# imjaegyun/Traffic-Context-Augmented-Vehicle-Trajectory-Prediction-Framework-Using-Multimodal-LLM

Hardware: AMD Instinct MI355X
Metric: trajectories/sec (higher is better)
Workload: dtype f16; 1 GPU; train.py step (:1168-1183): zero_grad + MultiModalTrajectoryModel.forward incl. loss (:914-964) + backward through the trainable part (LTSF + lane-polygon encoder; MLLM frozen, :1140-1145) + gradient all-reduce + AdamW(lr 5e-4, wd 1e-4); Llama-3.2-1B shape + LoRA r=8 + Q-Former + LTSF cross-attention head; dropout on as under ddp_model.train() (in-kernel Philox masks, regenerated in the backward); mode=train, variant=train.py (MLLM frozen), per_gpu_batch=32, global_batch=32, fused_seq_len=256, t_in=18, t_out=30, lora_r=8, parallelism=dp1, launch=eager

## Files before the change

traffic-context-augmented-vehicle-trajectory-prediction-framework-using-multimodal-llm_amd/csrc/gemm_bf16.hip:

```cpp
#include "gemm_params.hpp"
#include "gemm_epilogue.hpp"
#include "gemm_tile8.hpp"
#include "gemm_w4.hpp"
#include "gemm_skinny.hpp"
#include "gemm_splitk.hpp"

namespace tcavt {

template <int EPI, bool F16>
static int launch_small(const GemmP& p, int tile, int batch, hipStream_t stream) {
  GemmP q = p;
  q.prio = 0;
  const long wgs = (long)((q.M + 127) / 128) * ((q.N + 127) / 128) * batch;
  static const bool no_deep = getenv("TCAVT_GEMM_NO_DEEP") != nullptr;
  static const bool no_64 = getenv("TCAVT_GEMM_NO_64") != nullptr;
  if constexpr (EPI != EPI_ROPE && EPI != EPI_NORM && EPI != EPI_NORM16) {
    if ((tile == 64 || (tile == 0 && wgs <= 128 && !no_64)) && !no_deep) return launch<64, 64, 2, 2, EPI, F16, 2>(q, batch, stream);
  }
  if (wgs <= 256 && !no_deep) return launch<128, 128, 2, 2, EPI, F16, 2>(q, batch, stream);
  return launch<128, 128, 2, 2, EPI, F16, 1>(q, batch, stream);
}

template <int EPI, bool F16>
static int dispatch_tile(const GemmP& p, int tile, int batch, hipStream_t stream) {
// ... 51 lines not shown
}

extern "C" int tcavt_gemm_bf16(const tcavt_gemm_args* a, tcavt_stream_t stream) {
  TCAVT_CHECK_ARG(a != nullptr, "gemm_bf16: null args");
  const bool stream16 = (a->epilogue & TCAVT_EPI_NORM_OUT) && a->C == nullptr;
  TCAVT_CHECK_ARG(a->A && a->W && (a->C || stream16), "gemm_bf16: null A/W/C");
  TCAVT_CHECK_ARG(a->M > 0 && a->N > 0 && a->K > 0, "gemm_bf16: bad M/N/K %d/%d/%d", a->M, a->N, a->K);
  TCAVT_CHECK_ARG(a->K % 64 == 0, "gemm_bf16: K=%d must be a multiple of 64", a->K);
  TCAVT_CHECK_ARG(a->K < (1 << 26), "gemm_bf16: K too large");
  TCAVT_CHECK_ARG(a->N % 16 == 0, "gemm_bf16: N=%d must be a multiple of 16", a->N);
  TCAVT_CHECK_ARG(a->lda % 8 == 0 && a->ldw % 8 == 0 && a->lda >= a->K && a->ldw >= a->K,
                  "gemm_bf16: lda/ldw must be >= K and multiples of 8");
  TCAVT_CHECK_ARG(aligned16(a->A) && aligned16(a->W) && aligned16(a->C), "gemm_bf16: A/W/C must be 16-byte aligned");
  TCAVT_CHECK_ARG(a->out_dtype == TCAVT_F32 || a->out_dtype == TCAVT_BF16 || a->out_dtype == TCAVT_F16,
                  "gemm_bf16: bad out_dtype");
  TCAVT_CHECK_ARG(a->in_dtype == 0 || a->in_dtype == TCAVT_BF16 || a->in_dtype == TCAVT_F16, "gemm_bf16: bad in_dtype");
  const bool f16 = a->in_dtype == TCAVT_F16;
  const int batch = a->batch > 1 ? a->batch : 1;
  if (batch > 1)
    TCAVT_CHECK_ARG(!(a->epilogue & (TCAVT_EPI_SILU_MUL | TCAVT_EPI_ROPE)),
                    "gemm_bf16: batching is supported by the generic epilogue only");
  if (batch > 1) {
    TCAVT_CHECK_ARG(a->batch_inner >= 1 && batch % a->batch_inner == 0, "gemm_bf16: batch must be a multiple of batch_inner");
    TCAVT_CHECK_ARG(a->sAo % 8 == 0 && a->sAi % 8 == 0 && a->sWo % 8 == 0 && a->sWi % 8 == 0 && a->sCo % 4 == 0 &&
                        a->sCi % 4 == 0 && batch <= 65535,
                    "gemm_bf16: batch strides must keep 16-byte (A/W) and 4-element (C) alignment; batch <= 65535");
  }
  const int n_out = (a->epilogue & TCAVT_EPI_SILU_MUL) ? a->N / 2 : a->N;
  TCAVT_CHECK_ARG(a->ldc >= n_out && a->ldc % 4 == 0, "gemm_bf16: ldc=%ld too small or not a multiple of 4", (long)a->ldc);
  int K2 = 0;
  const bool lp_consumer = a->lora_part && (a->epilogue & TCAVT_EPI_ROPE);
  if ((a->A2 || a->W2 || a->K2) && !lp_consumer) {
    TCAVT_CHECK_ARG(a->A2 && a->W2 && a->K2 > 0 && a->K2 % 64 == 0,
                    "gemm_bf16: second K-source needs A2, W2 and K2 %% 64 == 0");
    TCAVT_CHECK_ARG(a->lda2 % 8 == 0 && a->ldw2 % 8 == 0 && a->lda2 >= a->K2 && a->ldw2 >= a->K2 &&
                        aligned16(a->A2) && aligned16(a->W2),
                    "gemm_bf16: bad lda2/ldw2/alignment");
    K2 = a->K2;
  }
  int epi = a->epilogue;
  if (epi & TCAVT_EPI_BIAS) TCAVT_CHECK_ARG(a->bias && aligned16(a->bias), "gemm_bf16: BIAS needs an aligned bias pointer");
  if (epi & TCAVT_EPI_BIAS_ROW) TCAVT_CHECK_ARG(a->bias && !(epi & TCAVT_EPI_BIAS), "gemm_bf16: BIAS_ROW needs bias and excludes BIAS");
  if ((epi & TCAVT_EPI_RESIDUAL) && !stream16)
    TCAVT_CHECK_ARG(a->residual && aligned16(a->residual) && a->ldr >= a->N && a->ldr % 4 == 0,
                    "gemm_bf16: RESIDUAL needs residual pointer and ldr >= N");
  if (epi & TCAVT_EPI_SILU_MUL)
    TCAVT_CHECK_ARG(a->N % 128 == 0 && !(epi & ~(TCAVT_EPI_SILU_MUL | TCAVT_EPI_ROWSCALE)),
                    "gemm_bf16: SILU_MUL needs N %% 128 == 0 and no other flag but ROWSCALE");
  if (epi & TCAVT_EPI_ROPE) {
    TCAVT_CHECK_ARG(a->N % 128 == 0 && !(epi & ~(TCAVT_EPI_ROPE | TCAVT_EPI_ROWSCALE)),
                    "gemm_bf16: ROPE needs N %% 128 == 0 and no other flag but ROWSCALE");
    TCAVT_CHECK_ARG(a->rope_cos && a->rope_sin && a->rope_L > 0 && a->rope_cols % 64 == 0 &&
                        aligned16(a->rope_cos) && aligned16(a->rope_sin),
                    "gemm_bf16: ROPE needs cos/sin tables, rope_L > 0, rope_cols %% 64 == 0");
  }
  TCAVT_CHECK_ARG(a->tile == 0 || a->tile == 64 || a->tile == 128 || a->tile == 256 || a->tile == 257 || a->tile == 271 || a->tile == 272,
                  "gemm_bf16: tile must be 0 (auto), 64, 128, 256, 257, 271 or 272");

  GemmP p;
  p.A = static_cast<const bf16_t*>(a->A);
  p.W = static_cast<const bf16_t*>(a->W);
  p.A2 = static_cast<const bf16_t*>(a->A2);
  p.W2 = static_cast<const bf16_t*>(a->W2);
  p.C = a->C;
  p.bias = a->bias;
  p.residual = a->residual;
  p.cosT = a->rope_cos;
  p.sinT = a->rope_sin;
  p.lda = a->lda; p.ldw = a->ldw; p.lda2 = a->lda2; p.ldw2 = a->ldw2; p.ldc = a->ldc; p.ldr = a->ldr;
  p.M = a->M; p.N = a->N; p.K = a->K; p.K2 = K2;
  p.out_kind = a->out_dtype;
  p.batch_inner = batch > 1 ? a->batch_inner : 1;
  p.w_group = a->batch_w_group > 1 ? a->batch_w_group : 1;
  p.sAo = a->sAo; p.sAi = a->sAi; p.sWo = a->sWo; p.sWi = a->sWi; p.sCo = a->sCo; p.sCi = a->sCi;
  p.flags = epi;
  p.rope_L = a->rope_L; p.rope_cols = a->rope_cols;
  p.tiles_m = p.tiles_n = 0;
  p.prio = 0;
  p.pers_tiles = 0;
  p.xcd_gx = 8;
  p.norm_h16 = nullptr;
  p.norm_part = nullptr;
  p.res16 = nullptr;
  p.lp_part = nullptr;
  p.lp_a = nullptr;
  p.lp_lda = 0;
  p.lp_np = 0;
  p.lp_scale = 1.f;
  p.w_frag = p.a_frag = p.o_frag = 0;
  if (a->act_layout != 0) {
    TCAVT_CHECK_ARG((a->act_layout & ~(TCAVT_ACT_A_FRAG16 | TCAVT_ACT_OUT_FRAG16 | TCAVT_ACT_BLOCK8)) == 0 && a->tile == 0 &&
                        skinny_shape(a->M, a->K) && batch == 1 && a->dropout_p == 0.f,
                    "gemm_bf16: act_layout (fragment-major activations) goes with the skinny form only (M <= 32, K %% 256 == 0, tile 0)");
    const int fmode = (a->act_layout & TCAVT_ACT_BLOCK8) ? 2 : 1;
    TCAVT_CHECK_ARG(fmode == 1 || a->M <= 8, "gemm_bf16: TCAVT_ACT_BLOCK8 holds at most 8 rows");
    p.a_frag = (a->act_layout & TCAVT_ACT_A_FRAG16) ? fmode : 0;
    if (a->act_layout & TCAVT_ACT_OUT_FRAG16) {
      const bool silu = (a->epilogue & ~TCAVT_EPI_ROWSCALE) == TCAVT_EPI_SILU_MUL && a->out_dtype == (f16 ? TCAVT_F16 : TCAVT_BF16) &&
                        a->N % 64 == 0;
      const bool stream = (a->epilogue & TCAVT_EPI_NORM_OUT) && stream16 && a->N % 32 == 0;
      TCAVT_CHECK_ARG(silu || stream, "gemm_bf16: TCAVT_ACT_OUT_FRAG16 needs SILU_MUL with a 16-bit output of the operand type, or "
                                      "NORM_OUT with C == NULL (the in-place 16-bit stream)");
      p.o_frag = fmode;
    }
  }
  if (a->w_layout != 0) {
    TCAVT_CHECK_ARG((a->w_layout == TCAVT_W_FRAG16 || a->w_layout == TCAVT_W_FRAG8) && a->tile == 0 && skinny_shape(a->M, a->K) && batch == 1 &&
                        a->dropout_p == 0.f && a->lda >= a->K && a->ldw == a->K && a->N % 16 == 0,
                    "gemm_bf16: w_layout = TCAVT_W_FRAG16 / TCAVT_W_FRAG8 (tcavt_pack_weight16 / tcavt_pack_weight8 copy) goes with the "
                    "skinny form only (M <= 32, K %% 256 == 0, N %% 16 == 0, tile 0, ldw == K)");
    p.w_frag = a->w_layout == TCAVT_W_FRAG8 ? 2 : 1;
  }
  if (a->lora_part) {
    TCAVT_CHECK_ARG(a->tile == 0 && skinny_shape(a->M, a->K) && batch == 1 && a->dropout_p == 0.f && aligned16(a->lora_part),
                    "gemm_bf16: lora_part goes with the skinny form only (M <= 32, tile 0)");
    p.lp_part = static_cast<float*>(a->lora_part);
    if (epi & TCAVT_EPI_NORM_OUT) {
      TCAVT_CHECK_ARG(a->lora_part_a && a->lora_part_lda >= a->N && a->lora_part_lda % 4 == 0 && ((uintptr_t)a->lora_part_a & 7) == 0,
                      "gemm_bf16: lora_part with NORM_OUT needs lora_part_a [32, lda >= N]");
      p.lp_a = static_cast<const bf16_t*>(a->lora_part_a);
      p.lp_lda = a->lora_part_lda;
    } else {
      TCAVT_CHECK_ARG((epi & TCAVT_EPI_ROPE) && a->lora_part_np > 0 && a->W2 && !a->A2 && a->K2 == 0 && a->ldw2 >= 32 && a->ldw2 % 8 == 0 &&
                          aligned16(a->W2) && a->M * 16 <= 512,
                      "gemm_bf16: lora_part with ROPE needs lora_part_np > 0, W2 (ldw2 >= 32) and no A2");
      p.lp_np = a->lora_part_np;
      p.lp_scale = a->lora_part_scale;
      p.W2 = static_cast<const bf16_t*>(a->W2);
      p.ldw2 = a->ldw2;
    }
  }
  p.sk_msplit = 1;
  p.sk_split = 1;
  p.sk_slab = nullptr;
  p.sk_cnt = nullptr;
  p.sk_slab_bytes = 0;
  p.sk_cnt_n = 0;
  if (a->splitk_ws && a->splitk_ws_bytes >= (64 << 10)) {
    TCAVT_CHECK_ARG(aligned16(a->splitk_ws), "gemm_bf16: splitk_ws must be 16-byte aligned");
    p.sk_cnt = static_cast<int*>(a->splitk_ws);
    p.sk_cnt_n = 4096;
    p.sk_slab = reinterpret_cast<float*>(static_cast<char*>(a->splitk_ws) + (16 << 10));
    p.sk_slab_bytes = a->splitk_ws_bytes - (16 << 10);
  }
  p.nf_flag = (epi & TCAVT_EPI_NORM_OUT) ? a->nonfinite_flag : nullptr;
  p.nf_tag = a->nonfinite_tag;
  p.norm_scale = 1.f;
  if (epi & TCAVT_EPI_NORM_OUT) {
    TCAVT_CHECK_ARG(a->norm_scale >= 0.f && a->norm_scale <= 1.f, "gemm_bf16: norm_scale must be in (0, 1] (0 means 1)");
    if (a->norm_scale != 0.f) p.norm_scale = a->norm_scale;
  }
  p.rs_part = nullptr;
  p.rope_pos = (epi & TCAVT_EPI_ROPE) ? a->rope_pos : nullptr;
  p.rs_npart = 0;
  p.rs_eps = p.rs_inv_h = 0.f;
  if (epi & TCAVT_EPI_NORM_OUT) {
    TCAVT_CHECK_ARG(!(epi & ~(TCAVT_EPI_NORM_OUT | TCAVT_EPI_RESIDUAL)) && a->out_dtype == TCAVT_F32 && batch == 1 && K2 == 0 &&
                        a->N % 64 == 0 && a->norm_h16 && a->norm_part && aligned16(a->norm_h16) && a->dropout_p == 0.f &&
                        (a->acc_scale == 0.f || a->acc_scale == 1.f) && a->tile != 64,
                    "gemm_bf16: NORM_OUT goes with an fp32 output (+ RESIDUAL) only, N %% 64 == 0, and needs norm_h16 / norm_part");
    TCAVT_CHECK_ARG(!stream16 || a->residual == nullptr,
                    "gemm_bf16: NORM_OUT with C == NULL keeps the residual stream in norm_h16 (updated in place): residual must be NULL");
    p.norm_h16 = static_cast<bf16_t*>(a->norm_h16);
    p.norm_part = a->norm_part;
    TCAVT_CHECK_ARG(a->norm_res16 == nullptr || (stream16 && aligned16(a->norm_res16)),
                    "gemm_bf16: norm_res16 goes with the 16-bit residual stream (NORM_OUT, C == NULL) and needs 16-byte alignment");
// ... 109 lines not shown
```

traffic-context-augmented-vehicle-trajectory-prediction-framework-using-multimodal-llm_amd/csrc/gemm_epilogue.hpp:

```cpp
#pragma once
#include "gemm_params.hpp"

namespace tcavt {

__device__ __forceinline__ void store_quad(const GemmP& p, int m, int n, f32x4 v) {
  if (p.out_kind == TCAVT_BF16) {
    u32x2 o = {pack_bf16x2(v[0], v[1]), pack_bf16x2(v[2], v[3])};
    *reinterpret_cast<u32x2*>(reinterpret_cast<bf16_t*>(p.C) + (long)m * p.ldc + n) = o;
  } else if (p.out_kind == TCAVT_F16) {
    u32x2 o = {pack_f16x2(v[0], v[1]), pack_f16x2(v[2], v[3])};
    *reinterpret_cast<u32x2*>(reinterpret_cast<bf16_t*>(p.C) + (long)m * p.ldc + n) = o;
  } else {
    *reinterpret_cast<f32x4*>(reinterpret_cast<float*>(p.C) + (long)m * p.ldc + n) = v;
  }
}

__device__ __forceinline__ float silu_mul(float g, float u) {
  return g * __builtin_amdgcn_rcpf(1.f + __expf(-g)) * u;
}

typedef __attribute__((ext_vector_type(2))) float f32x2;

template <bool F16>
__device__ __forceinline__ u32x2 silu_mul_quad(const f32x4& g, const f32x4& u) {
  const f32x2 g0 = {g[0], g[1]}, g1 = {g[2], g[3]}, u0 = {u[0], u[1]}, u1 = {u[2], u[3]};
  const f32x2 t0 = g0 * -1.44269504088896340736f, t1 = g1 * -1.44269504088896340736f;
  const f32x2 d0 = f32x2{__builtin_amdgcn_exp2f(t0[0]), __builtin_amdgcn_exp2f(t0[1])} + 1.f;
  const f32x2 d1 = f32x2{__builtin_amdgcn_exp2f(t1[0]), __builtin_amdgcn_exp2f(t1[1])} + 1.f;
  const f32x2 r0 = {__builtin_amdgcn_rcpf(d0[0]), __builtin_amdgcn_rcpf(d0[1])};
  const f32x2 r1 = {__builtin_amdgcn_rcpf(d1[0]), __builtin_amdgcn_rcpf(d1[1])};
  const f32x2 o0 = g0 * r0 * u0, o1 = g1 * r1 * u1;
  return u32x2{pack16x2<F16>(o0[0], o0[1]), pack16x2<F16>(o1[0], o1[1])};
}

__device__ __forceinline__ void swap16(unsigned& a, unsigned& b) {
  const auto r = __builtin_amdgcn_permlane16_swap(a, b, false, false);
  a = r[0];
  b = r[1];
}
__device__ __forceinline__ int pair16_off(int lane) {
  const int q = lane >> 4;
  return (q & 1) ? 16 + 4 * (q - 1) : 4 * q;
}
__device__ __forceinline__ void store_pair16(bf16_t* row_pair, int off, const u32x2& a, const u32x2& b) {
  unsigned a0 = a[0], a1 = a[1], b0 = b[0], b1 = b[1];
  swap16(a0, b0);
  swap16(a1, b1);
  *reinterpret_cast<u32x4*>(row_pair + off) = u32x4{a0, a1, b0, b1};
}
__device__ __forceinline__ void unswap_pair16(const u32x4& v, u32x2& a, u32x2& b) {
  unsigned a0 = v[0], a1 = v[1], b0 = v[2], b1 = v[3];
  swap16(a0, b0);
  swap16(a1, b1);
  a = u32x2{a0, a1};
  b = u32x2{b0, b1};
}

template <int TN, int TM>
__device__ __forceinline__ void pin_acc(f32x4 (&acc)[TN][TM], int i, int j) {
  asm volatile("" : "+a"(acc[i][j]));
}
template <int TM, int TN, int EPI, bool WHOLE_ONLY = false, bool F16 = false>
__device__ __forceinline__ void gemm_epilogue(const GemmP& p, f32x4 (&acc)[TN][TM], int m_base, int n_base, int lane,
                                              const float* rs_lds = nullptr) {
  constexpr int OUT16 = F16 ? TCAVT_F16 : TCAVT_BF16;
  float rsv[TM];
  if constexpr (EPI == EPI_SILU || EPI == EPI_SILU_SAVE || EPI == EPI_ROPE) {
    if (rs_lds) {
#pragma unroll
      for (int j = 0; j < TM; ++j) rsv[j] = rs_lds[j * 16 + (lane & 15)];
    } else if (p.rs_part) {
      float ss[TM];
      const f32x4* q[TM];
#pragma unroll
      for (int j = 0; j < TM; ++j) {
        ss[j] = 0.f;
        q[j] = reinterpret_cast<const f32x4*>(p.rs_part + (long)min(m_base + j * 16 + (lane & 15), p.M - 1) * p.rs_npart);
      }
      for (int i = 0; i < (p.rs_npart >> 2); ++i) {
#pragma unroll
        for (int j = 0; j < TM; ++j) {
          const f32x4 v = q[j][i];
          ss[j] += v[0];
          ss[j] += v[1];
          ss[j] += v[2];
          ss[j] += v[3];
        }
      }
#pragma unroll
      for (int j = 0; j < TM; ++j) rsv[j] = rsqrtf(ss[j] * p.rs_inv_h + p.rs_eps);
    } else {
#pragma unroll
      for (int j = 0; j < TM; ++j) rsv[j] = 1.f;
    }
  }
  const int nq = 4 * (lane >> 4);
  const int ml = lane & 15;
  const bool whole = WHOLE_ONLY || (m_base + TM * 16 <= p.M && n_base + TN * 16 <= p.N);
  if constexpr ((EPI == EPI_NORM || EPI == EPI_NORM16) && TN % 4 == 0) {
    const bool res = p.flags & TCAVT_EPI_RESIDUAL;
    const int npart = p.N >> 6;
    if constexpr (EPI == EPI_NORM16) {
      if constexpr (WHOLE_ONLY) {
        constexpr int DW = TM > 5 ? 5 : TM;
        const int off16 = pair16_off(lane);
        u32x4 oldw[TM][TN / 2];
        auto fetchw = [&](int j) {
          const bf16_t* hrow = p.res16 + (long)(m_base + j * 16 + ml) * p.ldc + n_base + off16;
#pragma unroll
          for (int k = 0; k < TN / 2; ++k)
            oldw[j][k] = res ? *reinterpret_cast<const u32x4*>(hrow + k * 32) : u32x4{0u, 0u, 0u, 0u};
        };
#pragma unroll
        for (int j = 0; j < DW; ++j) fetchw(j);
#pragma unroll
        for (int j = 0; j < TM; ++j) {
          if (j + DW < TM) fetchw(j + DW < TM ? j + DW : 0);
          const long m = m_base + j * 16 + ml;
          bf16_t* hrow = p.norm_h16 + m * p.ldc + n_base;
#pragma unroll
          for (int i = 0; i < TN; ++i) pin_acc(acc, i, j);
#pragma unroll
          for (int g = 0; g < TN / 4; ++g) {
            float ss = 0.f;
#pragma unroll
            for (int k = g * 2; k < g * 2 + 2; ++k) {
              u32x2 o[2], w[2];
              unswap_pair16(oldw[j][k], o[0], o[1]);
#pragma unroll
              for (int h = 0; h < 2; ++h) {
                const f32x4 v = fma4(acc[2 * k + h][j], p.norm_scale,
                                     f32x4{from16_lo<F16>(o[h][0]), from16_hi<F16>(o[h][0]), from16_lo<F16>(o[h][1]), from16_hi<F16>(o[h][1])});
                w[h] = u32x2{pack16x2<F16>(v[0], v[1]), pack16x2<F16>(v[2], v[3])};
                const float r0 = from16_lo<F16>(w[h][0]), r1 = from16_hi<F16>(w[h][0]), r2 = from16_lo<F16>(w[h][1]),
                            r3 = from16_hi<F16>(w[h][1]);
                ss += r0 * r0;
                ss += r1 * r1;
                ss += r2 * r2;
                ss += r3 * r3;
              }
              store_pair16(hrow + k * 32, off16, w[0], w[1]);
            }
            ss += __shfl_xor(ss, 16, 64);
            ss += __shfl_xor(ss, 32, 64);
            if (lane < 16) {
              p.norm_part[m * npart + ((n_base >> 6) + g)] = ss;
              flag_nonfinite(p, ss);
            }
          }
          __builtin_amdgcn_sched_barrier(0);
        }
        return;
      }
      constexpr int D = 1;
      u32x2 old[TM][TN];
      auto fetch = [&](int j) {
        const long m = m_base + j * 16 + ml;
        const long mm = m < p.M ? m : 0;
        const bf16_t* hrow = p.res16 + mm * p.ldc + n_base + nq;
#pragma unroll
        for (int i = 0; i < TN; ++i) {
          const bool colok = n_base + (i >> 2) * 64 < p.N;
          old[j][i] = (res && colok) ? *reinterpret_cast<const u32x2*>(hrow + i * 16) : u32x2{0u, 0u};
        }
      };
#pragma unroll
      for (int j = 0; j < D; ++j) fetch(j);
#pragma unroll
      for (int j = 0; j < TM; ++j) {
        if (j + D < TM) fetch(j + D < TM ? j + D : 0);
        const long m = m_base + j * 16 + ml;
        const bool rowok = m < p.M;
        const long mm = rowok ? m : 0;
        bf16_t* hrow = p.norm_h16 + mm * p.ldc + n_base + nq;
#pragma unroll
        for (int g = 0; g < TN / 4; ++g) {
          const bool colok = n_base + g * 64 < p.N;
          float ss = 0.f;
#pragma unroll
          for (int i = g * 4; i < g * 4 + 4; ++i) {
            const u32x2 o = old[j][i];
            const f32x4 v = fma4(acc[i][j], p.norm_scale,
                                 f32x4{from16_lo<F16>(o[0]), from16_hi<F16>(o[0]), from16_lo<F16>(o[1]), from16_hi<F16>(o[1])});
            const u32x2 w = u32x2{pack16x2<F16>(v[0], v[1]), pack16x2<F16>(v[2], v[3])};
            if (rowok && colok) *reinterpret_cast<u32x2*>(hrow + i * 16) = w;
            const float r0 = from16_lo<F16>(w[0]), r1 = from16_hi<F16>(w[0]), r2 = from16_lo<F16>(w[1]), r3 = from16_hi<F16>(w[1]);
            ss += r0 * r0;
            ss += r1 * r1;
            ss += r2 * r2;
            ss += r3 * r3;
          }
          ss += __shfl_xor(ss, 16, 64);
          ss += __shfl_xor(ss, 32, 64);
          if (lane < 16 && rowok && colok) {
            p.norm_part[m * npart + ((n_base >> 6) + g)] = ss;
            flag_nonfinite(p, ss);
          }
        }
      }
      return;
    } else {
      constexpr int D = WHOLE_ONLY ? 2 : 1;
      f32x4 rv[TM][TN];
      auto fetch = [&](int j) {
        const long m = m_base + j * 16 + ml;
        const long mm = (WHOLE_ONLY || m < p.M) ? m : 0;
        const float* rrow = p.residual + mm * p.ldr + n_base + nq;
#pragma unroll
        for (int i = 0; i < TN; ++i) {
          const bool colok = WHOLE_ONLY || n_base + (i >> 2) * 64 < p.N;
          rv[j][i] = (res && colok) ? *reinterpret_cast<const f32x4*>(rrow + i * 16) : f32x4{0.f, 0.f, 0.f, 0.f};
        }
      };
#pragma unroll
      for (int j = 0; j < D && j < TM; ++j) fetch(j);
#pragma unroll
      for (int j = 0; j < TM; ++j) {
        if (j + D < TM) fetch(j + D < TM ? j + D : 0);
        const long m = m_base + j * 16 + ml;
        const bool rowok = WHOLE_ONLY || m < p.M;
        const long mm = rowok ? m : 0;
        float* crow = reinterpret_cast<float*>(p.C) + mm * p.ldc + n_base + nq;
        bf16_t* hrow = p.norm_h16 + mm * p.ldc + n_base + nq;
        unsigned ovf = 0u;
#pragma unroll
        for (int g = 0; g < TN / 4; ++g) {
          const bool colok = WHOLE_ONLY || n_base + g * 64 < p.N;
          float ss = 0.f;
#pragma unroll
          for (int i = g * 4; i < g * 4 + 4; ++i) {
            const f32x4 vt = acc[i][j] + rv[j][i];
            const f32x4 v = vt * p.norm_scale;
            const u32x2 w = u32x2{pack16x2<F16>(v[0], v[1]), pack16x2<F16>(v[2], v[3])};
            if (rowok && colok) {
// ... 359 lines not shown
```

traffic-context-augmented-vehicle-trajectory-prediction-framework-using-multimodal-llm_amd/csrc/gemm_params.hpp:

```cpp
#pragma once
#include "common.hpp"
#include "philox.hpp"
#include <stdlib.h>

namespace tcavt {

struct GemmP {
  const bf16_t* A;
  const bf16_t* W;
  const bf16_t* A2;
  const bf16_t* W2;
  void* C;
  const float* bias;
  const float* residual;
  const float* cosT;
  const float* sinT;
  long lda, ldw, lda2, ldw2, ldc, ldr;
  int M, N, K, K2;
  int out_kind, flags, rope_L, rope_cols;
  int tiles_m, tiles_n;
  float acc_scale;
  int batch_inner;
  bf16_t* aux;
  long ldaux;
  int w_group;
  long sAo, sAi, sWo, sWi, sCo, sCi;
  int xcd_gx;
  DropoutP drop;
  int pers_tiles;
  int prio;
  bf16_t* norm_h16;
  float* norm_part;
  const float* rs_part;
  int rs_npart;
  float rs_eps, rs_inv_h;
  const int* rope_pos;
  const bf16_t* res16;
  float* lp_part;
  const bf16_t* lp_a;
  long lp_lda;
  int lp_np;
  float lp_scale;
  int sk_msplit;
  int a_frag, o_frag;
  int w_frag;
  int sk_split;
  float* sk_slab;
  int* sk_cnt;
  long sk_slab_bytes;
  int sk_cnt_n;
  int* nf_flag;
  int nf_tag;
  float norm_scale;
};

__device__ __forceinline__ f32x4 fma4(const f32x4& a, float s, const f32x4& b) {
  return __builtin_elementwise_fma(a, f32x4{s, s, s, s}, b);
}

__device__ __forceinline__ void flag_nonfinite(const GemmP& p, float ss) {
  if (p.nf_flag && !(ss <= 3.0e38f)) atomicCAS(p.nf_flag, 0, p.nf_tag);
}

__device__ __forceinline__ float row_rscale(const GemmP& p, long m) {
  const f32x4* q = reinterpret_cast<const f32x4*>(p.rs_part + m * p.rs_npart);
  float ss = 0.f;
  const int nq = p.rs_npart >> 2;
  for (int i0 = 0; i0 < nq; i0 += 8) {
    f32x4 v[8];
#pragma unroll
    for (int i = 0; i < 8; ++i) v[i] = q[min(i0 + i, nq - 1)];
#pragma unroll
    for (int i = 0; i < 8; ++i) {
      if (i0 + i < nq) {
        ss += v[i][0];
        ss += v[i][1];
        ss += v[i][2];
        ss += v[i][3];
      }
    }
  }
  return rsqrtf(ss * p.rs_inv_h + p.rs_eps);
}

enum { EPI_GENERIC = 0, EPI_SILU = 1, EPI_ROPE = 2, EPI_DROP = 3, EPI_SILU_SAVE = 4, EPI_NORM = 5, EPI_NORM16 = 6, EPI_SILUBWD = 7 };

__device__ __forceinline__ void glds16(const bf16_t* src, char* lds_wave_base) {
  __builtin_amdgcn_global_load_lds(
      (const __attribute__((address_space(1))) void*)src,
      (__attribute__((address_space(3))) void*)lds_wave_base, 16, 0, 0);
}

__device__ __forceinline__ void block_to_tile(const GemmP& p, int& tile_m, int& tile_n, int bid, int nwg) {
  constexpr int GM = 4;
  const int gx = p.xcd_gx;
  if (gx != 8) {
    const int gy = 8 / gx;
    const int xcd = bid & 7, local = bid >> 3;
    const int xi = xcd / gy, xj = xcd - xi * gy;
    const int sm = p.tiles_m / gx, sn = p.tiles_n / gy;
    const int per_group = GM * sn;
    const int g = local / per_group, in_g = local - g * per_group;
    const int gsz = min(GM, sm - g * GM);
    tile_m = xi * sm + g * GM + in_g % gsz;
    tile_n = xj * sn + in_g / gsz;
    return;
  }
  const int xcd = bid & 7, q = nwg >> 3, r = nwg & 7;
  const int wgid = (xcd < r ? xcd * (q + 1) : r * (q + 1) + (xcd - r) * q) + (bid >> 3);
  const int per_group = GM * p.tiles_n;
  const int g = wgid / per_group, in_g = wgid - g * per_group;
  const int gsz = min(GM, p.tiles_m - g * GM);
  tile_m = g * GM + in_g % gsz;
  tile_n = in_g / gsz;
}

__device__ __forceinline__ void block_to_tile(const GemmP& p, int& tile_m, int& tile_n) {
  block_to_tile(p, tile_m, tile_n, blockIdx.x, gridDim.x);
}

static int choose_xcd_partition(const GemmP& p) {
  static const int forced = [] {
    const char* e = getenv("TCAVT_GEMM_XCD_GX");
    return e ? atoi(e) : 0;
  }();
  const double a_bytes = (double)p.M * p.K, w_bytes = (double)p.N * p.K;
  int best = 8;
  double best_cost = 1.0 * a_bytes + 8.0 * w_bytes;
  for (int gx = 4; gx >= 1; gx /= 2) {
    const int gy = 8 / gx;
    if (p.tiles_m % gx || p.tiles_n % gy || (p.tiles_m / gx) % 4 || (long)p.tiles_m * p.tiles_n % 8) continue;
    if (forced == gx) return gx;
    const double cost = gy * a_bytes + gx * w_bytes;
    if (cost < best_cost) {
      best_cost = cost;
      best = gx;
// ... 7 lines not shown
```

traffic-context-augmented-vehicle-trajectory-prediction-framework-using-multimodal-llm_amd/csrc/gemm_w4.hpp:

```cpp
#pragma once
#include "gemm_epilogue.hpp"

namespace tcavt {

template <bool F16>
__device__ __forceinline__ void mfma_agpr(f32x4& c, const bf16x8& a, const bf16x8& b) {
  if constexpr (F16) asm volatile("v_mfma_f32_16x16x32_f16 %0, %1, %2, %0" : "+a"(c) : "v"(a), "v"(b));
  else asm volatile("v_mfma_f32_16x16x32_bf16 %0, %1, %2, %0" : "+a"(c) : "v"(a), "v"(b));
}

constexpr bool w4_pers_ok(int epi, bool deep) {
  return epi != EPI_ROPE && !(deep && epi == EPI_GENERIC);
}

template <int EPI, bool F16, int BN = 256, bool DEEP = false, int B2R = (BN == 256 ? 2 : 4)>
__global__ __launch_bounds__(256) void gemm_bf16_w4_kernel(GemmP p) {
  constexpr int BM = 256, NW = 4;
  constexpr int WN_ = BN == 256 ? 2 : 1, WM_ = NW / WN_;
  constexpr int TM = BM / WM_ / 16, TN = BN / WN_ / 16;
  static_assert(TM + TN == 16, "the fragment pipeline assumes 16 fragment loads per 32-deep K-step");
  constexpr int TILE_BYTES = (BM + BN) * 128;
  constexpr int NP = (BM + BN) / 32;
  constexpr int NB2 = B2R * TM;
  static_assert(!DEEP || (TM == 8 && TN == 8), "DEEP is laid out for the 2x2-wave form");
  constexpr int EARLY = NB2 / 4;
  constexpr int SPREAD = (TM * TN) / (NP - EARLY);
  extern __shared__ __attribute__((aligned(16))) char smem[];

  const int lane = threadIdx.x & 63;
  const int wave = __builtin_amdgcn_readfirstlane(threadIdx.x >> 6);
  const int wm = wave / WN_, wn = wave % WN_;
  constexpr bool RS = EPI == EPI_SILU || EPI == EPI_SILU_SAVE || EPI == EPI_ROPE;
  float* const rs_base = reinterpret_cast<float*>(smem + 2 * TILE_BYTES);
  int rs_sel = 0;
  constexpr bool PERS_OK = w4_pers_ok(EPI, DEEP);
  const bool pers = PERS_OK && p.pers_tiles > 0;
  const int total_tiles = pers ? p.pers_tiles : (int)gridDim.x;
  int vb = blockIdx.x;
  int tile_m, tile_n;
  block_to_tile(p, tile_m, tile_n, vb, total_tiles);
  int m0 = tile_m * BM, n0 = tile_n * BN;

  const int rl = lane >> 3;
  const int csw = (lane & 7) ^ (((wave & 1) * 4 + (rl >> 1)) & 7);
  const bf16_t* srcA = p.A + (long)(m0 + wave * 8 + rl) * p.lda + csw * 8;
  const bf16_t* srcW = p.W + (long)(n0 + wave * 8 + rl) * p.ldw + csw * 8;
  bool has_next = pers && vb + (int)gridDim.x < total_tiles;
  int nm0 = m0, nn0 = n0;
  const bf16_t* nxtA = srcA;
  const bf16_t* nxtW = srcW;
  auto locate_next = [&]() {
    if (has_next) {
      int tm, tn;
      block_to_tile(p, tm, tn, vb + (int)gridDim.x, total_tiles);
      nm0 = tm * BM;
      nn0 = tn * BN;
      nxtA = p.A + (long)(nm0 + wave * 8 + rl) * p.lda + csw * 8;
      nxtW = p.W + (long)(nn0 + wave * 8 + rl) * p.ldw + csw * 8;
    }
  };
  locate_next();
  const long stepA = 32 * p.lda, stepW = 32 * p.ldw;
  constexpr bool HASK2 = EPI == EPI_ROPE;
  const bf16_t* srcA2 = nullptr;
  const bf16_t* srcW2 = nullptr;
  long stepA2 = 0, stepW2 = 0;
  const int nt1 = p.K >> 6;
  int nt = nt1;
  auto locate_k2 = [&]() {
    if constexpr (HASK2) {
      if (p.K2 > 0) {
        srcA2 = p.A2 + (long)(m0 + wave * 8 + rl) * p.lda2 + csw * 8;
        srcW2 = p.W2 + (long)(n0 + wave * 8 + rl) * p.ldw2 + csw * 8;
      }
    }
  };
  if constexpr (HASK2) {
    if (p.K2 > 0) {
      stepA2 = 32 * p.lda2;
      stepW2 = 32 * p.ldw2;
      nt += p.K2 >> 6;
    }
  }
  locate_k2();

  struct Src {
    const bf16_t* a;
    const bf16_t* w;
    long sa, sw;
  };
  auto tsrc = [&](int t) -> Src {
    if constexpr (PERS_OK) {
      if (t >= nt && has_next) return Src{nxtA + (t - nt) * 64, nxtW + (t - nt) * 64, stepA, stepW};
    }
    t = min(t, nt - 1);
    if constexpr (HASK2) {
      if (t >= nt1) return Src{srcA2 + (t - nt1) * 64, srcW2 + (t - nt1) * 64, stepA2, stepW2};
    }
    return Src{srcA + t * 64, srcW + t * 64, stepA, stepW};
  };
  auto piece = [&](int buf, const Src& s, int r) {
    char* dst = smem + buf * TILE_BYTES + (r * NW + wave) * 1024;
    if (r < 8)
      glds16(s.a + r * s.sa, dst);
    else
      glds16(s.w + (r - 8) * s.sw, dst);
  };

  const int fsw = (lane >> 1) & 7;
  const int off0 = ((lane >> 4) ^ fsw) * 16;
  const int off1 = ((4 + (lane >> 4)) ^ fsw) * 16;
  const int xrow = (wm * TM * 16 + (lane & 15)) * 128;
  const int wrow = (BM + wn * TN * 16 + (lane & 15)) * 128;

  f32x4 acc[TN][TM];
#pragma unroll
  for (int i = 0; i < TN; ++i)
#pragma unroll
    for (int j = 0; j < TM; ++j) acc[i][j] = f32x4{0.f, 0.f, 0.f, 0.f};

  bf16x8 w0[TN], x0[TM], w1[TN], x1[TM];
  auto ldx = [&](const char* base, int off, int j) { return *reinterpret_cast<const bf16x8*>(base + xrow + j * 2048 + off); };
  auto ldw = [&](const char* base, int off, int i) { return *reinterpret_cast<const bf16x8*>(base + wrow + i * 2048 + off); };

  if constexpr (RS) {
    if (p.rs_part) rs_base[threadIdx.x] = row_rscale(p, m0 + threadIdx.x);
  }
  {
    const Src s0 = tsrc(0);
#pragma unroll
    for (int r = 0; r < NP; ++r) piece(0, s0, r);
  }
  __syncthreads();
  Src sn1 = tsrc(1);
  if constexpr (DEEP) {
#pragma unroll
    for (int r = 0; r < NP; ++r) piece(1, sn1, r);
  } else if (nt > 1) {
#pragma unroll
    for (int r = 0; r < EARLY; ++r) piece(1, sn1, r);
  }
#pragma unroll
  for (int j = 0; j < TM; ++j) x0[j] = ldx(smem, off0, j);
#pragma unroll
  for (int i = 0; i < TN; ++i) w0[i] = ldw(smem, off0, i);

  int cur = 0;
  auto ktile = [&](int t) {
    const char* base = smem + cur * TILE_BYTES;
    const char* nbase = smem + (cur ^ 1) * TILE_BYTES;
    Src sn2;
    int koff2 = 0;
    bool second2 = false, into_next2 = false;
#pragma unroll
    for (int i = 0; i < TN; ++i) {
#pragma unroll
      for (int j = 0; j < TM; ++j) {
        mfma_agpr<F16>(acc[i][j], w0[i], x0[j]);
        const int idx = i * TM + j;
        if (idx < 32 && (idx & 1) == 0) {
          const int f = idx >> 1;
          if (f < TM) x1[f] = ldx(base, off1, f);
          else w1[f - TM] = ldw(base, off1, f - TM);
        }
        if constexpr (DEEP) {
          if (idx == 0) {
            into_next2 = PERS_OK && has_next && t + 2 >= nt;
            const int tt = into_next2 ? t + 2 - nt : min(t + 2, nt - 1);
            second2 = HASK2 && !into_next2 && tt >= nt1;
            koff2 = (second2 ? tt - nt1 : tt) * 64;
          }
          if (idx == 3) sn2.a = (into_next2 ? nxtA : second2 ? srcA2 : srcA) + koff2;
          if (idx == 6) sn2.w = (into_next2 ? nxtW : second2 ? srcW2 : srcW) + koff2;
          if (idx == 9) {
            sn2.sa = second2 ? stepA2 : stepA;
            sn2.sw = second2 ? stepW2 : stepW;
          }
          if (idx == 39) asm volatile("s_waitcnt lgkmcnt(0)\n\ts_barrier" ::: "memory");
          if (idx >= 43 && (idx & 3) == 3) piece(cur, sn2, (idx - 43) / 4);
        } else {
          if (idx % SPREAD == SPREAD - 1 && EARLY + idx / SPREAD < NP) piece(cur ^ 1, sn1, EARLY + idx / SPREAD);
        }
      }
    }
#pragma unroll
    for (int i = 0; i < TN - B2R; ++i)
#pragma unroll
      for (int j = 0; j < TM; ++j) {
        mfma_agpr<F16>(acc[i][j], w1[i], x1[j]);
        const int idx = i * TM + j;
        if constexpr (DEEP) {
          if ((idx & 3) == 3 && 6 + idx / 4 < NP) piece(cur, sn2, 6 + idx / 4);
          continue;
        }
        if (idx == 0) {
          into_next2 = PERS_OK && has_next && t + 2 >= nt;
          const int tt = into_next2 ? t + 2 - nt : min(t + 2, nt - 1);
          second2 = HASK2 && !into_next2 && tt >= nt1;
          koff2 = (second2 ? tt - nt1 : tt) * 64;
        }
        if (idx == 3) sn2.a = (into_next2 ? nxtA : second2 ? srcA2 : srcA) + koff2;
        if (idx == 6) sn2.w = (into_next2 ? nxtW : second2 ? srcW2 : srcW) + koff2;
        if (idx == 9) {
          sn2.sa = second2 ? stepA2 : stepA;
          sn2.sw = second2 ? stepW2 : stepW;
        }
      }
    if (DEEP) asm volatile("s_waitcnt vmcnt(%0) lgkmcnt(0)\n\ts_barrier" ::"n"(NP) : "memory");
    else __syncthreads();
#pragma unroll
    for (int i = TN - B2R; i < TN; ++i) {
#pragma unroll
      for (int j = 0; j < TM; ++j) {
        mfma_agpr<F16>(acc[i][j], w1[i], x1[j]);
        const int idx = (i - (TN - B2R)) * TM + j;
        if (TM == TN && idx < TM) {
          x0[idx] = ldx(nbase, off0, idx);
          w0[idx] = ldw(nbase, off0, idx);
        }
        if (TM != TN && idx < 16) {
          if (idx < TM) x0[idx] = ldx(nbase, off0, idx);
          else w0[idx - TM] = ldw(nbase, off0, idx - TM);
        }
        if (!DEEP && (idx & 3) == 3 && (idx >> 2) < EARLY) piece(cur, sn2, idx >> 2);
      }
    }
    if (t == nt - 1) asm volatile("s_nop 15\n\ts_nop 15" ::: "memory");
    cur ^= 1;
    sn1 = sn2;
  };
  for (;;) {
    for (int t = 0; t < nt; ++t) ktile(t);
    asm volatile("s_nop 15\n\ts_nop 15" ::: "memory");
#pragma unroll
    for (int i = 0; i < TN; ++i)
#pragma unroll
      for (int j = 0; j < TM; ++j) asm volatile("" : "+a"(acc[i][j]));
    const int em0 = m0, en0 = n0;
    const bool cont = PERS_OK && has_next;
    if (cont) {
      vb += gridDim.x;
      if constexpr (RS) {
        if (p.rs_part) rs_base[(rs_sel ^ 1) * 256 + threadIdx.x] = row_rscale(p, nm0 + threadIdx.x);
      }
      m0 = nm0;
      n0 = nn0;
      srcA = nxtA;
      srcW = nxtW;
      locate_k2();
      has_next = vb + (int)gridDim.x < total_tiles;
      locate_next();
    }
    __builtin_amdgcn_sched_barrier(0);
    gemm_epilogue<TM, TN, EPI, true, F16>(p, acc, em0 + wm * TM * 16, en0 + wn * TN * 16, lane,
                                          (RS && p.rs_part) ? rs_base + rs_sel * 256 + wm * TM * 16 : nullptr);
    if (!cont) {
      if constexpr (DEEP) asm volatile("s_waitcnt vmcnt(0)" ::: "memory");
      break;
    }
    rs_sel ^= 1;
#pragma unroll
    for (int i = 0; i < TN; ++i)
#pragma unroll
      for (int j = 0; j < TM; ++j) {
        acc[i][j] = f32x4{0.f, 0.f, 0.f, 0.f};
        asm volatile("" : "+a"(acc[i][j]));
      }
    asm volatile("s_nop 7" ::: "memory");
  }
}

template <bool F16>
static bool silu16_ok(const GemmP& p) {
  return p.out_kind == (F16 ? TCAVT_F16 : TCAVT_BF16) && (p.ldc & 7) == 0;
}

template <int EPI, bool F16, int BN = 256, bool DEEP = false>
static int launch_w4(const GemmP& p0, hipStream_t stream) {
  if constexpr (EPI == EPI_SILU || EPI == EPI_SILU_SAVE) {
    if (!silu16_ok<F16>(p0)) {
      set_error("gemm_bf16(w4): the SiLU epilogue of the 4-wave kernel writes the 16-bit operand type with ldc %% 8 == 0");
      return TCAVT_ERR_ARG;
    }
  }
  if constexpr (EPI == EPI_SILUBWD) {
    if (p0.out_kind != (F16 ? TCAVT_F16 : TCAVT_BF16) || (p0.ldc & 7) || (p0.ldaux & 7) || p0.aux == nullptr || p0.ldc < 2 * p0.N ||
        p0.ldaux < 2 * p0.N) {
      set_error("gemm_bf16(w4): SILU_BWD needs silu_preact, 16-bit output of the operand type, ldc / ld_preact %% 8 == 0 and >= 2 N");
      return TCAVT_ERR_ARG;
    }
  }
  if constexpr (EPI == EPI_ROPE) {
    if (p0.ldc & 7) {
      set_error("gemm_bf16(w4): the RoPE epilogue of the 4-wave kernel needs ldc %% 8 == 0");
      return TCAVT_ERR_ARG;
    }
  }
  if constexpr (EPI == EPI_NORM16) {
    if (p0.ldc & 7) {
      set_error("gemm_bf16(w4): the in-place 16-bit residual epilogue of the 4-wave kernel needs ldc %% 8 == 0");
      return TCAVT_ERR_ARG;
    }
  }
  GemmP p = p0;
  p.tiles_m = p.M / 256;
  p.tiles_n = p.N / BN;
  p.xcd_gx = choose_xcd_partition(p);
  constexpr int lds = 2 * (256 + BN) * 128 + 2048;
  auto kfn = gemm_bf16_w4_kernel<EPI, F16, BN, DEEP>;
  static bool attr_set = false;
  if (!attr_set) {
    hipError_t e = hipFuncSetAttribute(reinterpret_cast<const void*>(kfn),
                                       hipFuncAttributeMaxDynamicSharedMemorySize, lds);
    if (e != hipSuccess) {
      set_error("gemm_bf16(w4): hipFuncSetAttribute(%d B LDS) failed: %s", lds, hipGetErrorString(e));
      return TCAVT_ERR_HIP;
    }
    attr_set = true;
  }
  const int tiles = p.tiles_m * p.tiles_n;
  static const bool no_pers = getenv("TCAVT_GEMM_NO_PERSIST") != nullptr;
  static const int n_cu = [] {
    int dev = 0, n = 0;
    if (hipGetDevice(&dev) != hipSuccess || hipDeviceGetAttribute(&n, hipDeviceAttributeMultiprocessorCount, dev) != hipSuccess) n = 256;
    return n / 8 * 8;
  }();
  int wgs = tiles;
  p.pers_tiles = 0;
  if (w4_pers_ok(EPI, DEEP) && !no_pers && n_cu >= 8 && tiles > n_cu && p.K + p.K2 >= 128) {
    p.pers_tiles = tiles;
    wgs = n_cu;
  }
  dim3 grid(wgs), block(256);
  hipLaunchKernelGGL(kfn, grid, block, lds, stream, p);
  TCAVT_CHECK_LAUNCH("gemm_bf16(w4)");
  return TCAVT_OK;
}

}
```

Baseline: 2141 trajectories/sec.

## Prefetch residual tile into LDS through the k-loop pipeline for NORM16 epilogue

For the w4 GEMM with the NORM16 epilogue and a residual, on a workgroup's last tile the freed k-loop load pipeline streams the residual rows into LDS as extra pseudo k-tiles. The epilogue then reads the residual from LDS with a shallower prefetch depth instead of issuing global loads. This targets residual-read latency in the fused residual+norm epilogue. It adds addressing complexity, a barrier before the epilogue, and a runtime flag (default on) to disable it.

```diff
diff --git a/traffic-context-augmented-vehicle-trajectory-prediction-framework-using-multimodal-llm_amd/csrc/gemm_bf16.hip b/traffic-context-augmented-vehicle-trajectory-prediction-framework-using-multimodal-llm_amd/csrc/gemm_bf16.hip
--- a/traffic-context-augmented-vehicle-trajectory-prediction-framework-using-multimodal-llm_amd/csrc/gemm_bf16.hip
+++ b/traffic-context-augmented-vehicle-trajectory-prediction-framework-using-multimodal-llm_amd/csrc/gemm_bf16.hip
@@ -157,6 +157,7 @@
   p.norm_h16 = nullptr;
   p.norm_part = nullptr;
   p.res16 = nullptr;
+  p.res_pf = 0;
   p.lp_part = nullptr;
   p.lp_a = nullptr;
   p.lp_lda = 0;
diff --git a/traffic-context-augmented-vehicle-trajectory-prediction-framework-using-multimodal-llm_amd/csrc/gemm_epilogue.hpp b/traffic-context-augmented-vehicle-trajectory-prediction-framework-using-multimodal-llm_amd/csrc/gemm_epilogue.hpp
--- a/traffic-context-augmented-vehicle-trajectory-prediction-framework-using-multimodal-llm_amd/csrc/gemm_epilogue.hpp
+++ b/traffic-context-augmented-vehicle-trajectory-prediction-framework-using-multimodal-llm_amd/csrc/gemm_epilogue.hpp
@@ -60,9 +60,13 @@
 __device__ __forceinline__ void pin_acc(f32x4 (&acc)[TN][TM], int i, int j) {
   asm volatile("" : "+a"(acc[i][j]));
 }
+template <int V>
+struct int_c {
+  static constexpr int value = V;
+};
 template <int TM, int TN, int EPI, bool WHOLE_ONLY = false, bool F16 = false>
 __device__ __forceinline__ void gemm_epilogue(const GemmP& p, f32x4 (&acc)[TN][TM], int m_base, int n_base, int lane,
-                                              const float* rs_lds = nullptr) {
+                                              const float* rs_lds = nullptr, const char* res_lds = nullptr, int res_half = 0) {
   constexpr int OUT16 = F16 ? TCAVT_F16 : TCAVT_BF16;
   float rsv[TM];
   if constexpr (EPI == EPI_SILU || EPI == EPI_SILU_SAVE || EPI == EPI_ROPE) {
@@ -102,7 +106,6 @@
     const int npart = p.N >> 6;
     if constexpr (EPI == EPI_NORM16) {
       if constexpr (WHOLE_ONLY) {
-        constexpr int DW = TM > 5 ? 5 : TM;
         const int off16 = pair16_off(lane);
         u32x4 oldw[TM][TN / 2];
         auto fetchw = [&](int j) {
@@ -111,11 +114,18 @@
           for (int k = 0; k < TN / 2; ++k)
             oldw[j][k] = res ? *reinterpret_cast<const u32x4*>(hrow + k * 32) : u32x4{0u, 0u, 0u, 0u};
         };
-#pragma unroll
-        for (int j = 0; j < DW; ++j) fetchw(j);
+        auto fetchl = [&](int j) {
+#pragma unroll
+          for (int k = 0; k < TN / 2; ++k)
+            oldw[j][k] = *reinterpret_cast<const u32x4*>(res_lds + (k >> 1) * res_half + j * 8192 + (k & 1) * 512);
+        };
+        auto rows = [&](auto fetch, auto depth) {
+        constexpr int DW = decltype(depth)::value;
+#pragma unroll
+        for (int j = 0; j < DW; ++j) fetch(j);
 #pragma unroll
         for (int j = 0; j < TM; ++j) {
-          if (j + DW < TM) fetchw(j + DW < TM ? j + DW : 0);
+          if (j + DW < TM) fetch(j + DW < TM ? j + DW : 0);
           const long m = m_base + j * 16 + ml;
           bf16_t* hrow = p.norm_h16 + m * p.ldc + n_base;
 #pragma unroll
@@ -150,6 +160,9 @@
           }
           __builtin_amdgcn_sched_barrier(0);
         }
+        };
+        if (res_lds) rows(fetchl, int_c<(TM > 2 ? 2 : TM)>{});
+        else rows(fetchw, int_c<(TM > 5 ? 5 : TM)>{});
         return;
       }
       constexpr int D = 1;
diff --git a/traffic-context-augmented-vehicle-trajectory-prediction-framework-using-multimodal-llm_amd/csrc/gemm_params.hpp b/traffic-context-augmented-vehicle-trajectory-prediction-framework-using-multimodal-llm_amd/csrc/gemm_params.hpp
--- a/traffic-context-augmented-vehicle-trajectory-prediction-framework-using-multimodal-llm_amd/csrc/gemm_params.hpp
+++ b/traffic-context-augmented-vehicle-trajectory-prediction-framework-using-multimodal-llm_amd/csrc/gemm_params.hpp
@@ -52,6 +52,7 @@
   int* nf_flag;
   int nf_tag;
   float norm_scale;
+  int res_pf;
 };
 
 __device__ __forceinline__ f32x4 fma4(const f32x4& a, float s, const f32x4& b) {
diff --git a/traffic-context-augmented-vehicle-trajectory-prediction-framework-using-multimodal-llm_amd/csrc/gemm_w4.hpp b/traffic-context-augmented-vehicle-trajectory-prediction-framework-using-multimodal-llm_amd/csrc/gemm_w4.hpp
--- a/traffic-context-augmented-vehicle-trajectory-prediction-framework-using-multimodal-llm_amd/csrc/gemm_w4.hpp
+++ b/traffic-context-augmented-vehicle-trajectory-prediction-framework-using-multimodal-llm_amd/csrc/gemm_w4.hpp
@@ -45,6 +45,7 @@
   const int csw = (lane & 7) ^ (((wave & 1) * 4 + (rl >> 1)) & 7);
   const bf16_t* srcA = p.A + (long)(m0 + wave * 8 + rl) * p.lda + csw * 8;
   const bf16_t* srcW = p.W + (long)(n0 + wave * 8 + rl) * p.ldw + csw * 8;
+  const long stepA = 32 * p.lda, stepW = 32 * p.ldw;
   bool has_next = pers && vb + (int)gridDim.x < total_tiles;
   int nm0 = m0, nn0 = n0;
   const bf16_t* nxtA = srcA;
@@ -60,11 +61,26 @@
     }
   };
   locate_next();
-  const long stepA = 32 * p.lda, stepW = 32 * p.ldw;
   constexpr bool HASK2 = EPI == EPI_ROPE;
   const bf16_t* srcA2 = nullptr;
   const bf16_t* srcW2 = nullptr;
   long stepA2 = 0, stepW2 = 0;
+  constexpr bool RPF = EPI == EPI_NORM16 && BN == 256;
+  const bool rpf = RPF && p.res_pf;
+  bool tail_res = false;
+  long nstepA = 0, nstepW = 0;
+  auto locate_res = [&]() {
+    if constexpr (RPF) {
+      tail_res = rpf && !has_next;
+      nstepA = stepA;
+      nstepW = stepW;
+      if (tail_res) {
+        nxtA = p.res16 + (long)(m0 + wm * 128 + (lane & 7)) * p.ldc + n0 + wn * 128 + (lane >> 5) * 32 + pair16_off(((lane >> 3) & 3) << 4);
+        nxtW = nxtA + 64 * p.ldc;
+        nstepA = nstepW = 8 * p.ldc;
+      }
+    }
+  };
   const int nt1 = p.K >> 6;
   int nt = nt1;
   auto locate_k2 = [&]() {
@@ -83,6 +99,7 @@
     }
   }
   locate_k2();
+  locate_res();
 
   struct Src {
     const bf16_t* a;
@@ -91,7 +108,11 @@
   };
   auto tsrc = [&](int t) -> Src {
     if constexpr (PERS_OK) {
-      if (t >= nt && has_next) return Src{nxtA + (t - nt) * 64, nxtW + (t - nt) * 64, stepA, stepW};
+      if constexpr (RPF) {
+        if (t >= nt && (has_next || tail_res)) return Src{nxtA + (t - nt) * 64, nxtW + (t - nt) * 64, nstepA, nstepW};
+      } else {
+        if (t >= nt && has_next) return Src{nxtA + (t - nt) * 64, nxtW + (t - nt) * 64, stepA, stepW};
+      }
     }
     t = min(t, nt - 1);
     if constexpr (HASK2) {
@@ -136,7 +157,7 @@
   if constexpr (DEEP) {
 #pragma unroll
     for (int r = 0; r < NP; ++r) piece(1, sn1, r);
-  } else if (nt > 1) {
+  } else if (nt > 1 || (RPF && tail_res)) {
 #pragma unroll
     for (int r = 0; r < EARLY; ++r) piece(1, sn1, r);
   }
@@ -165,7 +186,7 @@
         }
         if constexpr (DEEP) {
           if (idx == 0) {
-            into_next2 = PERS_OK && has_next && t + 2 >= nt;
+            into_next2 = PERS_OK && (has_next || (RPF && tail_res)) && t + 2 >= nt;
             const int tt = into_next2 ? t + 2 - nt : min(t + 2, nt - 1);
             second2 = HASK2 && !into_next2 && tt >= nt1;
             koff2 = (second2 ? tt - nt1 : tt) * 64;
@@ -173,8 +194,8 @@
           if (idx == 3) sn2.a = (into_next2 ? nxtA : second2 ? srcA2 : srcA) + koff2;
           if (idx == 6) sn2.w = (into_next2 ? nxtW : second2 ? srcW2 : srcW) + koff2;
           if (idx == 9) {
-            sn2.sa = second2 ? stepA2 : stepA;
-            sn2.sw = second2 ? stepW2 : stepW;
+            sn2.sa = second2 ? stepA2 : (RPF && into_next2) ? nstepA : stepA;
+            sn2.sw = second2 ? stepW2 : (RPF && into_next2) ? nstepW : stepW;
           }
           if (idx == 39) asm volatile("s_waitcnt lgkmcnt(0)\n\ts_barrier" ::: "memory");
           if (idx >= 43 && (idx & 3) == 3) piece(cur, sn2, (idx - 43) / 4);
@@ -194,7 +215,7 @@
           continue;
         }
         if (idx == 0) {
-          into_next2 = PERS_OK && has_next && t + 2 >= nt;
+          into_next2 = PERS_OK && (has_next || (RPF && tail_res)) && t + 2 >= nt;
           const int tt = into_next2 ? t + 2 - nt : min(t + 2, nt - 1);
           second2 = HASK2 && !into_next2 && tt >= nt1;
           koff2 = (second2 ? tt - nt1 : tt) * 64;
@@ -202,8 +223,8 @@
         if (idx == 3) sn2.a = (into_next2 ? nxtA : second2 ? srcA2 : srcA) + koff2;
         if (idx == 6) sn2.w = (into_next2 ? nxtW : second2 ? srcW2 : srcW) + koff2;
         if (idx == 9) {
-          sn2.sa = second2 ? stepA2 : stepA;
-          sn2.sw = second2 ? stepW2 : stepW;
+          sn2.sa = second2 ? stepA2 : (RPF && into_next2) ? nstepA : stepA;
+          sn2.sw = second2 ? stepW2 : (RPF && into_next2) ? nstepW : stepW;
         }
       }
     if (DEEP) asm volatile("s_waitcnt vmcnt(%0) lgkmcnt(0)\n\ts_barrier" ::"n"(NP) : "memory");
@@ -231,6 +252,13 @@
   };
   for (;;) {
     for (int t = 0; t < nt; ++t) ktile(t);
+    const bool from_lds = RPF && tail_res;
+    if constexpr (RPF && !DEEP) {
+      if (from_lds) {
+#pragma unroll
+        for (int r = EARLY; r < NP; ++r) piece(cur ^ 1, sn1, r);
+      }
+    }
     asm volatile("s_nop 15\n\ts_nop 15" ::: "memory");
 #pragma unroll
     for (int i = 0; i < TN; ++i)
@@ -250,10 +278,19 @@
       locate_k2();
       has_next = vb + (int)gridDim.x < total_tiles;
       locate_next();
+      locate_res();
     }
     __builtin_amdgcn_sched_barrier(0);
+    const char* res_lds = nullptr;
+    if constexpr (RPF) {
+      if (from_lds) {
+        asm volatile("s_waitcnt vmcnt(0)\n\ts_barrier" ::: "memory");
+        res_lds = smem + cur * TILE_BYTES + (((lane >> 3) & 1) * NW + wave) * 1024 + ((lane >> 4) * 8 + (lane & 7)) * 16;
+      }
+    }
     gemm_epilogue<TM, TN, EPI, true, F16>(p, acc, em0 + wm * TM * 16, en0 + wn * TN * 16, lane,
-                                          (RS && p.rs_part) ? rs_base + rs_sel * 256 + wm * TM * 16 : nullptr);
+                                          (RS && p.rs_part) ? rs_base + rs_sel * 256 + wm * TM * 16 : nullptr, res_lds,
+                                          (cur ^ 1) * TILE_BYTES - cur * TILE_BYTES);
     if (!cont) {
       if constexpr (DEEP) asm volatile("s_waitcnt vmcnt(0)" ::: "memory");
       break;
@@ -331,6 +368,11 @@
     p.pers_tiles = tiles;
     wgs = n_cu;
   }
+  p.res_pf = 0;
+  if constexpr (EPI == EPI_NORM16 && BN == 256) {
+    const char* e = getenv("TCAVT_GEMM_NO_RES_PREFETCH");
+    p.res_pf = (p.flags & TCAVT_EPI_RESIDUAL) && !(e && e[0] && e[0] != '0');
+  }
   dim3 grid(wgs), block(256);
   hipLaunchKernelGGL(kfn, grid, block, lds, stream, p);
   TCAVT_CHECK_LAUNCH("gemm_bf16(w4)");
```

Result: faster. 2163 trajectories/sec, median of 6 (+1.0%).
